# yoxu515/aot-benchmark

Hardware: NVIDIA H100
Metric: frames/sec (480p, 10 obj) (higher is better)
Workload: dtype f32

## Files before the change

aot_benchmark_b200/csrc/attn_tc.cuh:

```cuda
#pragma once
#include "common.cuh"
#include "tc_common.cuh"

namespace aotb {
namespace tc {

constexpr float AT_LOG2E = 1.4426950408889634f;

struct AttnTcArgs {
    int N, Tk;
    const int* Tk_dev;
    float* O;
    int ldo;
    float* Opart;
    float* Mpart;
    float* Lpart;
    int splits;
    int split_unit;
    int spin;
    float* dbg;
};

template <int QC, int VC, int STAGES, int BK, int NWG>
struct AttnSmem {
    static constexpr int BM = 64 * NWG;
    static constexpr int Q_BYTES = QC * BM * 128;
    static constexpr int K_BYTES = QC * BK * 128;
    static constexpr int V_BYTES = VC * BK * 128;
    static constexpr int STAGE_BYTES = K_BYTES + V_BYTES;
    static constexpr int TOTAL = Q_BYTES + STAGES * STAGE_BYTES + (1 + 2 * STAGES) * 8 + 1024;
};

template <int N>
__device__ __forceinline__ void wgmma_ss(float* d, uint64_t a, uint64_t b, uint32_t scale_d) {
    if (N == 128) wgmma_ss_n128(d, a, b, scale_d);
    else wgmma_ss_n64(d, a, b, scale_d);
}

template <int QC, int VC, int STAGES, bool EXACT, int BK, int NWG, bool AHEAD>
__global__ void __launch_bounds__(32 * (4 * NWG + 1), NWG == 1 ? 2 : 1)
attn_tc_kernel(const __grid_constant__ CUtensorMap tmQ, const __grid_constant__ CUtensorMap tmK,
               const __grid_constant__ CUtensorMap tmV, const AttnTcArgs a) {
    using SM = AttnSmem<QC, VC, STAGES, BK, NWG>;
    constexpr int BM = SM::BM, TMA_WARP = 4 * NWG, SR = BK / 2;
    extern __shared__ uint8_t smem_raw[];
    uint8_t* smem = reinterpret_cast<uint8_t*>((reinterpret_cast<uintptr_t>(smem_raw) + 1023) & ~(uintptr_t)1023);
    uint8_t* sQ = smem;
    uint8_t* sKV = smem + SM::Q_BYTES;
    uint64_t* q_full = reinterpret_cast<uint64_t*>(sKV + STAGES * SM::STAGE_BYTES);
    uint64_t* kv_full = q_full + 1;
    uint64_t* kv_free = kv_full + STAGES;

    const int tid = threadIdx.x, warp = tid >> 5, lane = tid & 31;
    const int qt = blockIdx.x, y = blockIdx.y, z = blockIdx.z;
    const int qc0 = QC == 1 ? y : 0, vc0 = y * VC;
    pdl_trigger();
    if (tid == 0) {
        mbar_init(q_full, 1);
        for (int s = 0; s < STAGES; ++s) { mbar_init(&kv_full[s], 1); mbar_init(&kv_free[s], 4 * NWG); }
        fence_mbar_init();
    }
    __syncthreads();
    pdl_wait();

    const int tk = a.Tk_dev ? *a.Tk_dev : a.Tk;
    const int units = (tk + a.split_unit - 1) / a.split_unit;
    const int per = (units + a.splits - 1) / a.splits;
    const int k0 = min(z * per * a.split_unit, tk), k1 = min((z + 1) * per * a.split_unit, tk);
    const int ntiles = (k1 - k0 + BK - 1) / BK;

    if (warp == TMA_WARP) {
        if (elect_one() && ntiles > 0) {
            tma_prefetch_desc(&tmQ); tma_prefetch_desc(&tmK); tma_prefetch_desc(&tmV);
            mbar_arrive_expect_tx(q_full, SM::Q_BYTES);
            for (int c = 0; c < QC; ++c) tma_load_3d(sQ + c * BM * 128, &tmQ, q_full, 0, qt * BM, qc0 + c);
            for (int n = 0; n < ntiles; ++n) {
                const int s = n % STAGES;
                if (n >= STAGES) mbar_wait(&kv_free[s], ((n / STAGES) - 1) & 1);
                uint8_t* st = sKV + s * SM::STAGE_BYTES;
                mbar_arrive_expect_tx(&kv_full[s], SM::STAGE_BYTES);
                const int key0 = k0 + n * BK;
                for (int c = 0; c < QC; ++c) tma_load_3d(st + c * BK * 128, &tmK, &kv_full[s], 0, key0, qc0 + c);
                for (int v = 0; v < VC; ++v)
                    tma_load_3d(st + SM::K_BYTES + v * BK * 128, &tmV, &kv_full[s], 0, key0, vc0 + v);
            }
        }
        return;
    }

    const int wg = warp >> 2, wq = warp & 3;
    const int row0 = wg * 64 + wq * 16 + (lane >> 2);
    const int cq = (lane & 3) * 2;
    float m[2] = {-INFINITY, -INFINITY}, l[2] = {0.f, 0.f};
    float o[VC][32];
#pragma unroll
    for (int v = 0; v < VC; ++v)
#pragma unroll
        for (int j = 0; j < 32; ++j) o[v][j] = 0.f;
    const bool dump = a.dbg && blockIdx.x == 0 && blockIdx.y == 0 && blockIdx.z == 0;
    const uint64_t dQ = smem_desc_sw128(smem_u32(sQ + wg * 64 * 128));
    const uint64_t dKV0 = smem_desc_sw128(smem_u32(sKV));
    if (ntiles > 0) mbar_wait_cp(q_full, 0, a.spin);

    auto issue_s = [&](int n, float* sc) {
        const uint64_t dK = dKV0 + (uint64_t)(((n % STAGES) * SM::STAGE_BYTES) >> 4);
        wgmma_fence();
#pragma unroll
        for (int c = 0; c < QC; ++c) {
            const uint64_t q = dQ + (uint64_t)((c * BM * 128) >> 4), k = dK + (uint64_t)((c * BK * 128) >> 4);
#pragma unroll
            for (int ks = 0; ks < 2; ++ks) {
                wgmma_ss<BK>(sc, q + 2 * ks, k + 2 * ks, (c | ks) ? 1u : 0u);
                if (EXACT) {
                    wgmma_ss<BK>(sc, q + 4 + 2 * ks, k + 2 * ks, 1u);
                    wgmma_ss<BK>(sc, q + 2 * ks, k + 4 + 2 * ks, 1u);
                }
            }
        }
        wgmma_commit();
    };
    float sbuf[AHEAD ? 2 : 1][SR];
    if (AHEAD && ntiles > 0) {
        mbar_wait_cp(&kv_full[0], 0, a.spin);
        issue_s(0, sbuf[0]);
    }

#pragma unroll 1
    for (int n = 0; n < ntiles; ++n) {
        const int s = n % STAGES;
        float* sc = sbuf[0];
        if (AHEAD) {
            if (n + 1 < ntiles) {
                mbar_wait_cp(&kv_full[(n + 1) % STAGES], ((n + 1) / STAGES) & 1, a.spin);
                issue_s(n + 1, sbuf[AHEAD ? 1 : 0]);
                wgmma_wait<1>();
            } else {
                wgmma_wait<0>();
            }
        } else {
            mbar_wait_cp(&kv_full[s], (n / STAGES) & 1, a.spin);
            issue_s(n, sc);
            wgmma_wait<0>();
        }
        reg_fence<SR>(sc);
        const uint64_t dV = dKV0 + (uint64_t)((s * SM::STAGE_BYTES + SM::K_BYTES) >> 4);
        const int key0 = k0 + n * BK;
        if (dump && key0 < 128) {
#pragma unroll
            for (int j = 0; j < SR; ++j) {
                const int key = key0 + 8 * (j >> 2) + cq + (j & 1);
                if (key < 128) a.dbg[(row0 + 8 * ((j >> 1) & 1)) * 128 + key] = sc[j];
            }
        }
        if (key0 + BK > k1) {
#pragma unroll
            for (int j = 0; j < SR; ++j)
                if (key0 + 8 * (j >> 2) + cq + (j & 1) >= k1) sc[j] = -INFINITY;
        }
        float mx[2] = {m[0], m[1]};
#pragma unroll
        for (int j = 0; j < SR; ++j) mx[(j >> 1) & 1] = fmaxf(mx[(j >> 1) & 1], sc[j]);
#pragma unroll
        for (int h = 0; h < 2; ++h) {
            mx[h] = fmaxf(mx[h], __shfl_xor_sync(0xffffffffu, mx[h], 1));
            mx[h] = fmaxf(mx[h], __shfl_xor_sync(0xffffffffu, mx[h], 2));
        }
        float f[2], neg[2];
#pragma unroll
        for (int h = 0; h < 2; ++h) {
            f[h] = mx[h] > m[h] ? ex2((m[h] - mx[h]) * AT_LOG2E) : 1.f;
            m[h] = mx[h];
            l[h] *= f[h];
            neg[h] = m[h] * AT_LOG2E;
        }
#pragma unroll
        for (int v = 0; v < VC; ++v)
#pragma unroll
            for (int j = 0; j < 32; ++j) o[v][j] *= f[(j >> 1) & 1];
        uint32_t ph[SR / 2], pl[SR / 2];
#pragma unroll
        for (int j = 0; j < SR; j += 2) {
            const int h = (j >> 1) & 1;
            const float p0 = ex2(fmaf(sc[j], AT_LOG2E, -neg[h])), p1 = ex2(fmaf(sc[j + 1], AT_LOG2E, -neg[h]));
            l[h] += p0 + p1;
            const __half2 hi = __floats2half2_rn(p0, p1);
            ph[j >> 1] = *reinterpret_cast<const uint32_t*>(&hi);
            if (EXACT) pl[j >> 1] = cvt_h2(p0 - __low2float(hi), p1 - __high2float(hi));
        }
        wgmma_fence();
#pragma unroll
        for (int v = 0; v < VC; ++v) {
            const uint64_t vd = dV + (uint64_t)((v * BK * 128) >> 4);
#pragma unroll
            for (int kk = 0; kk < BK / 16; ++kk) {
                wgmma_rs_n64_tb(o[v], ph + 4 * kk, vd + (uint64_t)(kk * 128));
                if (EXACT) wgmma_rs_n64_tb(o[v], pl + 4 * kk, vd + (uint64_t)(kk * 128));
            }
        }
        wgmma_commit();
        wgmma_wait<0>();
#pragma unroll
        for (int v = 0; v < VC; ++v) reg_fence<32>(o[v]);
        mbar_arrive_warp(&kv_free[s]);
        if (AHEAD) {
            reg_fence<SR>(sbuf[AHEAD ? 1 : 0]);
#pragma unroll
            for (int j = 0; j < SR; ++j) sbuf[0][j] = sbuf[AHEAD ? 1 : 0][j];
        }
    }

#pragma unroll
    for (int h = 0; h < 2; ++h) {
        l[h] += __shfl_xor_sync(0xffffffffu, l[h], 1);
        l[h] += __shfl_xor_sync(0xffffffffu, l[h], 2);
    }
    if (dump) {
#pragma unroll
        for (int j = 0; j < 32; ++j) a.dbg[128 * 128 + (row0 + 8 * ((j >> 1) & 1)) * 64 + 8 * (j >> 2) + cq + (j & 1)] = o[0][j];
    }
    const int cols = gridDim.y * VC * 32;
#pragma unroll
    for (int h = 0; h < 2; ++h) {
        const int q = qt * BM + row0 + 8 * h;
        if (q >= a.N) continue;
        const float inv = 1.f / l[h];
#pragma unroll
        for (int v = 0; v < VC; ++v) {
#pragma unroll
            for (int g = 0; g < 4; ++g) {
                const int j = 4 * g + 2 * h;
                float2 r = make_float2(o[v][j] + o[v][j + 16], o[v][j + 1] + o[v][j + 17]);
                const int col = (vc0 + v) * 32 + 8 * g + cq;
                if (a.splits == 1) {
                    r.x *= inv; r.y *= inv;
                    *reinterpret_cast<float2*>(a.O + (size_t)q * a.ldo + col) = r;
                } else {
                    *reinterpret_cast<float2*>(a.Opart + ((size_t)z * a.N + q) * cols + col) = r;
                }
            }
        }
        if (a.splits > 1 && (lane & 3) == 0 && (QC == 1 || y == 0)) {
            const size_t idx = ((size_t)z * (QC == 1 ? gridDim.y : 1) + (QC == 1 ? y : 0)) * a.N + q;
            a.Mpart[idx] = m[h];
            a.Lpart[idx] = l[h];
        }
    }
}

template <int QC, int VC, int STAGES, int BK, int NWG, bool AHEAD>
int launch_attn_tc(const CUtensorMap& tq, const CUtensorMap& tk, const CUtensorMap& tv, const AttnTcArgs& a, dim3 grid,
                   int exact, cudaStream_t st, const char* what) {
    constexpr int smem = AttnSmem<QC, VC, STAGES, BK, NWG>::TOTAL;
    auto kt = attn_tc_kernel<QC, VC, STAGES, true, BK, NWG, AHEAD>;
    auto kf = attn_tc_kernel<QC, VC, STAGES, false, BK, NWG, AHEAD>;
    static bool configured = false;
    if (!configured) {
        cudaError_t e = cudaFuncSetAttribute(kt, cudaFuncAttributeMaxDynamicSharedMemorySize, smem);
        if (e == cudaSuccess) e = cudaFuncSetAttribute(kf, cudaFuncAttributeMaxDynamicSharedMemorySize, smem);
        if (e != cudaSuccess) {
            set_error("%s: cudaFuncSetAttribute: %s", what, cudaGetErrorString(e));
            return AOTB_ERR_CUDA;
        }
        configured = true;
    }
    launch(exact ? kt : kf, grid, dim3(32 * (4 * NWG + 1)), smem, st, tq, tk, tv, a);
    return check_launch(what);
}

}
}
```

aot_benchmark_b200/csrc/tc_common.cuh:

```cuda
#pragma once
#include <cuda.h>
#include <cuda_fp16.h>
#include <cuda_runtime.h>
#include <cstdint>

namespace aotb {
namespace tc {

__device__ __forceinline__ uint32_t smem_u32(const void* p) { return (uint32_t)__cvta_generic_to_shared(p); }

__device__ __forceinline__ bool elect_one() {
    uint32_t pred;
    asm volatile(
        "{\n\t.reg .pred P;\n\telect.sync _|P, 0xffffffff;\n\tselp.b32 %0, 1, 0, P;\n\t}\n" : "=r"(pred));
    return pred != 0;
}

__device__ __forceinline__ void mbar_init(uint64_t* bar, uint32_t count) {
    asm volatile("mbarrier.init.shared::cta.b64 [%0], %1;" ::"r"(smem_u32(bar)), "r"(count) : "memory");
}
__device__ __forceinline__ void fence_mbar_init() { asm volatile("fence.mbarrier_init.release.cluster;" ::: "memory"); }
__device__ __forceinline__ void mbar_arrive_warp(uint64_t* bar) {
    __syncwarp();
    if ((threadIdx.x & 31) == 0) asm volatile("mbarrier.arrive.shared::cta.b64 _, [%0];" ::"r"(smem_u32(bar)) : "memory");
}
__device__ __forceinline__ void mbar_arrive(uint64_t* bar) {
    asm volatile("mbarrier.arrive.shared::cta.b64 _, [%0];" ::"r"(smem_u32(bar)) : "memory");
}
__device__ __forceinline__ void mbar_arrive_expect_tx(uint64_t* bar, uint32_t bytes) {
    asm volatile("mbarrier.arrive.expect_tx.shared::cta.b64 _, [%0], %1;" ::"r"(smem_u32(bar)), "r"(bytes) : "memory");
}
__device__ __forceinline__ void mbar_wait(uint64_t* bar, uint32_t parity) {
    const uint32_t addr = smem_u32(bar);
    uint32_t done = 0;
    uint32_t spins = 0;
    while (true) {
        asm volatile(
            "{\n\t.reg .pred P;\n\tmbarrier.try_wait.parity.shared::cta.b64 P, [%1], %2, %3;\n\tselp.b32 %0, 1, 0, P;\n\t}\n"
            : "=r"(done)
            : "r"(addr), "r"(parity), "r"(20000u)
            : "memory");
        if (done) break;
        if (++spins > (1u << 24)) __trap();
    }
}

__device__ __forceinline__ void mbar_wait_spin(uint64_t* bar, uint32_t parity) {
    const uint32_t addr = smem_u32(bar);
    uint32_t done = 0;
    uint32_t spins = 0;
    while (true) {
        asm volatile(
            "{\n\t.reg .pred P;\n\tmbarrier.try_wait.parity.shared::cta.b64 P, [%1], %2;\n\tselp.b32 %0, 1, 0, P;\n\t}\n"
            : "=r"(done)
            : "r"(addr), "r"(parity)
            : "memory");
        if (done) break;
        if (++spins > (1u << 28)) __trap();
    }
}

__device__ __forceinline__ void mbar_wait_cp(uint64_t* bar, uint32_t parity, int spin) {
    if (spin) mbar_wait_spin(bar, parity);
    else mbar_wait(bar, parity);
}

__device__ __forceinline__ void tma_prefetch_desc(const CUtensorMap* m) {
    asm volatile("prefetch.tensormap [%0];" ::"l"(reinterpret_cast<uint64_t>(m)) : "memory");
}
__device__ __forceinline__ void tma_load_2d(void* dst, const CUtensorMap* m, uint64_t* bar, int c0, int c1) {
    asm volatile(
        "cp.async.bulk.tensor.2d.shared::cluster.global.mbarrier::complete_tx::bytes [%0], [%1, {%3, %4}], [%2];"
        ::"r"(smem_u32(dst)), "l"(reinterpret_cast<uint64_t>(m)), "r"(smem_u32(bar)), "r"(c0), "r"(c1)
        : "memory");
}
__device__ __forceinline__ void tma_load_3d(void* dst, const CUtensorMap* m, uint64_t* bar, int c0, int c1, int c2) {
    asm volatile(
        "cp.async.bulk.tensor.3d.shared::cluster.global.mbarrier::complete_tx::bytes [%0], [%1, {%3, %4, %5}], [%2];"
        ::"r"(smem_u32(dst)), "l"(reinterpret_cast<uint64_t>(m)), "r"(smem_u32(bar)), "r"(c0), "r"(c1), "r"(c2)
        : "memory");
}
__device__ __forceinline__ void fence_proxy_async() { asm volatile("fence.proxy.async.shared::cta;" ::: "memory"); }

__device__ __forceinline__ uint64_t smem_desc_sw128(uint32_t saddr) {
    uint64_t d = 0;
    d |= (uint64_t)((saddr & 0x3FFFF) >> 4);
    d |= (uint64_t)1 << 16;
    d |= (uint64_t)(1024 >> 4) << 32;
    d |= (uint64_t)1 << 62;
    return d;
}
__device__ __forceinline__ void wgmma_fence() { asm volatile("wgmma.fence.sync.aligned;" ::: "memory"); }
__device__ __forceinline__ void wgmma_commit() { asm volatile("wgmma.commit_group.sync.aligned;" ::: "memory"); }
template <int N>
__device__ __forceinline__ void wgmma_wait() { asm volatile("wgmma.wait_group.sync.aligned %0;" ::"n"(N) : "memory"); }
template <int R>
__device__ __forceinline__ void reg_fence(float* d) {
#pragma unroll
    for (int i = 0; i < R; ++i) asm volatile("" : "+f"(d[i])::"memory");
}

__device__ __forceinline__ void wgmma_ss_n64(float* d, uint64_t a_desc, uint64_t b_desc, uint32_t scale_d) {
    asm volatile(
        "{\n\t.reg .pred p;\n\tsetp.ne.b32 p, %34, 0;\n\t"
        "wgmma.mma_async.sync.aligned.m64n64k16.f32.f16.f16 "
        "{%0, %1, %2, %3, %4, %5, %6, %7, %8, %9, %10, %11, %12, %13, %14, %15, "
        "%16, %17, %18, %19, %20, %21, %22, %23, %24, %25, %26, %27, %28, %29, %30, %31}, "
        "%32, %33, p, 1, 1, 0, 0;\n\t}\n"
        : "+f"(d[0]), "+f"(d[1]), "+f"(d[2]), "+f"(d[3]), "+f"(d[4]), "+f"(d[5]), "+f"(d[6]), "+f"(d[7]),
          "+f"(d[8]), "+f"(d[9]), "+f"(d[10]), "+f"(d[11]), "+f"(d[12]), "+f"(d[13]), "+f"(d[14]), "+f"(d[15]),
          "+f"(d[16]), "+f"(d[17]), "+f"(d[18]), "+f"(d[19]), "+f"(d[20]), "+f"(d[21]), "+f"(d[22]), "+f"(d[23]),
          "+f"(d[24]), "+f"(d[25]), "+f"(d[26]), "+f"(d[27]), "+f"(d[28]), "+f"(d[29]), "+f"(d[30]), "+f"(d[31])
        : "l"(a_desc), "l"(b_desc), "r"(scale_d));
}

__device__ __forceinline__ void wgmma_ss_n128(float* d, uint64_t a_desc, uint64_t b_desc, uint32_t scale_d) {
    asm volatile(
        "{\n\t.reg .pred p;\n\tsetp.ne.b32 p, %66, 0;\n\t"
        "wgmma.mma_async.sync.aligned.m64n128k16.f32.f16.f16 "
        "{%0, %1, %2, %3, %4, %5, %6, %7, %8, %9, %10, %11, %12, %13, %14, %15, "
        "%16, %17, %18, %19, %20, %21, %22, %23, %24, %25, %26, %27, %28, %29, %30, %31, "
        "%32, %33, %34, %35, %36, %37, %38, %39, %40, %41, %42, %43, %44, %45, %46, %47, "
        "%48, %49, %50, %51, %52, %53, %54, %55, %56, %57, %58, %59, %60, %61, %62, %63}, "
        "%64, %65, p, 1, 1, 0, 0;\n\t}\n"
        : "+f"(d[0]), "+f"(d[1]), "+f"(d[2]), "+f"(d[3]), "+f"(d[4]), "+f"(d[5]), "+f"(d[6]), "+f"(d[7]),
          "+f"(d[8]), "+f"(d[9]), "+f"(d[10]), "+f"(d[11]), "+f"(d[12]), "+f"(d[13]), "+f"(d[14]), "+f"(d[15]),
          "+f"(d[16]), "+f"(d[17]), "+f"(d[18]), "+f"(d[19]), "+f"(d[20]), "+f"(d[21]), "+f"(d[22]), "+f"(d[23]),
          "+f"(d[24]), "+f"(d[25]), "+f"(d[26]), "+f"(d[27]), "+f"(d[28]), "+f"(d[29]), "+f"(d[30]), "+f"(d[31]),
          "+f"(d[32]), "+f"(d[33]), "+f"(d[34]), "+f"(d[35]), "+f"(d[36]), "+f"(d[37]), "+f"(d[38]), "+f"(d[39]),
          "+f"(d[40]), "+f"(d[41]), "+f"(d[42]), "+f"(d[43]), "+f"(d[44]), "+f"(d[45]), "+f"(d[46]), "+f"(d[47]),
          "+f"(d[48]), "+f"(d[49]), "+f"(d[50]), "+f"(d[51]), "+f"(d[52]), "+f"(d[53]), "+f"(d[54]), "+f"(d[55]),
          "+f"(d[56]), "+f"(d[57]), "+f"(d[58]), "+f"(d[59]), "+f"(d[60]), "+f"(d[61]), "+f"(d[62]), "+f"(d[63])
        : "l"(a_desc), "l"(b_desc), "r"(scale_d));
}

__device__ __forceinline__ void wgmma_ss_n256(float* d, uint64_t a_desc, uint64_t b_desc, uint32_t scale_d) {
    asm volatile(
        "{\n\t.reg .pred p;\n\tsetp.ne.b32 p, %130, 0;\n\t"
        "wgmma.mma_async.sync.aligned.m64n256k16.f32.f16.f16 "
        "{%0, %1, %2, %3, %4, %5, %6, %7, %8, %9, %10, %11, %12, %13, %14, %15, "
        "%16, %17, %18, %19, %20, %21, %22, %23, %24, %25, %26, %27, %28, %29, %30, %31, "
        "%32, %33, %34, %35, %36, %37, %38, %39, %40, %41, %42, %43, %44, %45, %46, %47, "
        "%48, %49, %50, %51, %52, %53, %54, %55, %56, %57, %58, %59, %60, %61, %62, %63, "
        "%64, %65, %66, %67, %68, %69, %70, %71, %72, %73, %74, %75, %76, %77, %78, %79, "
        "%80, %81, %82, %83, %84, %85, %86, %87, %88, %89, %90, %91, %92, %93, %94, %95, "
        "%96, %97, %98, %99, %100, %101, %102, %103, %104, %105, %106, %107, %108, %109, %110, %111, "
        "%112, %113, %114, %115, %116, %117, %118, %119, %120, %121, %122, %123, %124, %125, %126, %127}, "
        "%128, %129, p, 1, 1, 0, 0;\n\t}\n"
        : "+f"(d[0]), "+f"(d[1]), "+f"(d[2]), "+f"(d[3]), "+f"(d[4]), "+f"(d[5]), "+f"(d[6]), "+f"(d[7]),
          "+f"(d[8]), "+f"(d[9]), "+f"(d[10]), "+f"(d[11]), "+f"(d[12]), "+f"(d[13]), "+f"(d[14]), "+f"(d[15]),
          "+f"(d[16]), "+f"(d[17]), "+f"(d[18]), "+f"(d[19]), "+f"(d[20]), "+f"(d[21]), "+f"(d[22]), "+f"(d[23]),
          "+f"(d[24]), "+f"(d[25]), "+f"(d[26]), "+f"(d[27]), "+f"(d[28]), "+f"(d[29]), "+f"(d[30]), "+f"(d[31]),
          "+f"(d[32]), "+f"(d[33]), "+f"(d[34]), "+f"(d[35]), "+f"(d[36]), "+f"(d[37]), "+f"(d[38]), "+f"(d[39]),
          "+f"(d[40]), "+f"(d[41]), "+f"(d[42]), "+f"(d[43]), "+f"(d[44]), "+f"(d[45]), "+f"(d[46]), "+f"(d[47]),
          "+f"(d[48]), "+f"(d[49]), "+f"(d[50]), "+f"(d[51]), "+f"(d[52]), "+f"(d[53]), "+f"(d[54]), "+f"(d[55]),
          "+f"(d[56]), "+f"(d[57]), "+f"(d[58]), "+f"(d[59]), "+f"(d[60]), "+f"(d[61]), "+f"(d[62]), "+f"(d[63]),
          "+f"(d[64]), "+f"(d[65]), "+f"(d[66]), "+f"(d[67]), "+f"(d[68]), "+f"(d[69]), "+f"(d[70]), "+f"(d[71]),
          "+f"(d[72]), "+f"(d[73]), "+f"(d[74]), "+f"(d[75]), "+f"(d[76]), "+f"(d[77]), "+f"(d[78]), "+f"(d[79]),
          "+f"(d[80]), "+f"(d[81]), "+f"(d[82]), "+f"(d[83]), "+f"(d[84]), "+f"(d[85]), "+f"(d[86]), "+f"(d[87]),
          "+f"(d[88]), "+f"(d[89]), "+f"(d[90]), "+f"(d[91]), "+f"(d[92]), "+f"(d[93]), "+f"(d[94]), "+f"(d[95]),
          "+f"(d[96]), "+f"(d[97]), "+f"(d[98]), "+f"(d[99]), "+f"(d[100]), "+f"(d[101]), "+f"(d[102]), "+f"(d[103]),
          "+f"(d[104]), "+f"(d[105]), "+f"(d[106]), "+f"(d[107]), "+f"(d[108]), "+f"(d[109]), "+f"(d[110]), "+f"(d[111]),
          "+f"(d[112]), "+f"(d[113]), "+f"(d[114]), "+f"(d[115]), "+f"(d[116]), "+f"(d[117]), "+f"(d[118]), "+f"(d[119]),
          "+f"(d[120]), "+f"(d[121]), "+f"(d[122]), "+f"(d[123]), "+f"(d[124]), "+f"(d[125]), "+f"(d[126]), "+f"(d[127])
        : "l"(a_desc), "l"(b_desc), "r"(scale_d));
}

__device__ __forceinline__ void wgmma_rs_n64_tb(float* d, const uint32_t* a, uint64_t b_desc) {
    asm volatile(
        "{\n\t.reg .pred p;\n\tsetp.ne.b32 p, 1, 0;\n\t"
        "wgmma.mma_async.sync.aligned.m64n64k16.f32.f16.f16 "
        "{%0, %1, %2, %3, %4, %5, %6, %7, %8, %9, %10, %11, %12, %13, %14, %15, "
        "%16, %17, %18, %19, %20, %21, %22, %23, %24, %25, %26, %27, %28, %29, %30, %31}, "
        "{%32, %33, %34, %35}, %36, p, 1, 1, 1;\n\t}\n"
        : "+f"(d[0]), "+f"(d[1]), "+f"(d[2]), "+f"(d[3]), "+f"(d[4]), "+f"(d[5]), "+f"(d[6]), "+f"(d[7]),
          "+f"(d[8]), "+f"(d[9]), "+f"(d[10]), "+f"(d[11]), "+f"(d[12]), "+f"(d[13]), "+f"(d[14]), "+f"(d[15]),
          "+f"(d[16]), "+f"(d[17]), "+f"(d[18]), "+f"(d[19]), "+f"(d[20]), "+f"(d[21]), "+f"(d[22]), "+f"(d[23]),
          "+f"(d[24]), "+f"(d[25]), "+f"(d[26]), "+f"(d[27]), "+f"(d[28]), "+f"(d[29]), "+f"(d[30]), "+f"(d[31])
        : "r"(a[0]), "r"(a[1]), "r"(a[2]), "r"(a[3]), "l"(b_desc));
}


__device__ __forceinline__ float ex2(float x) {
    float y;
    asm("ex2.approx.ftz.f32 %0, %1;" : "=f"(y) : "f"(x));
    return y;
}
__device__ __forceinline__ uint32_t cvt_h2(float lo, float hi) {
    uint32_t r;
    asm("cvt.rn.f16x2.f32 %0, %1, %2;" : "=r"(r) : "f"(hi), "f"(lo));
    return r;
}

__device__ __forceinline__ void cluster_sync_all() {
    asm volatile("barrier.cluster.arrive.release.aligned;\n\tbarrier.cluster.wait.acquire.aligned;" ::: "memory");
}
__device__ __forceinline__ uint32_t dsmem_addr(uint32_t local_saddr, uint32_t cta_rank) {
    uint32_t r;
    asm volatile("mapa.shared::cluster.u32 %0, %1, %2;" : "=r"(r) : "r"(local_saddr), "r"(cta_rank));
    return r;
}
__device__ __forceinline__ float4 dsmem_ld_f4(uint32_t cluster_saddr) {
    float4 v;
    asm volatile("ld.shared::cluster.v4.f32 {%0, %1, %2, %3}, [%4];"
                 : "=f"(v.x), "=f"(v.y), "=f"(v.z), "=f"(v.w)
                 : "r"(cluster_saddr));
    return v;
}

typedef CUresult (*PFN_encodeTiled)(CUtensorMap*, CUtensorMapDataType, cuuint32_t, void*, const cuuint64_t*,
                                    const cuuint64_t*, const cuuint32_t*, const cuuint32_t*, CUtensorMapInterleave,
                                    CUtensorMapSwizzle, CUtensorMapL2promotion, CUtensorMapFloatOOBfill);
PFN_encodeTiled tensor_map_encoder();

int make_tmap_rows64(CUtensorMap* out, const void* base, int rows, int heads, int box_rows);

}
}
```

Before: 362.3.

## Add FA3-style intra-warpgroup softmax/GEMM pipelining with ping-pong warpgroup scheduling

For the QC=1, VC=1, BK=64, NWG=2 non-AHEAD configuration, the attention loop is restructured so each step issues the next tile's QK^T GEMM and the current tile's PV GEMM together. The softmax and exp/pack for the next tile then runs while the PV GEMM is in flight, with P fragments double-buffered in registers. Named barriers make the two warpgroups take turns issuing tensor-core work, so one warpgroup's softmax overlaps the other's GEMMs. The intent is to hide softmax latency behind tensor-core work, at the cost of more register pressure and extra barrier synchronisation. The row-sum rescale is folded into the exp accumulation.

Result: faster. 367.9, median of 6 (+1.5%).

```diff
diff --git a/aot_benchmark_b200/csrc/attn_tc.cuh b/aot_benchmark_b200/csrc/attn_tc.cuh
--- a/aot_benchmark_b200/csrc/attn_tc.cuh
+++ b/aot_benchmark_b200/csrc/attn_tc.cuh
@@ -43,6 +43,7 @@
                const __grid_constant__ CUtensorMap tmV, const AttnTcArgs a) {
     using SM = AttnSmem<QC, VC, STAGES, BK, NWG>;
     constexpr int BM = SM::BM, TMA_WARP = 4 * NWG, SR = BK / 2;
+    constexpr bool PIPE = QC == 1 && VC == 1 && BK == 64 && NWG == 2 && !AHEAD;
     extern __shared__ uint8_t smem_raw[];
     uint8_t* smem = reinterpret_cast<uint8_t*>((reinterpret_cast<uintptr_t>(smem_raw) + 1023) & ~(uintptr_t)1023);
     uint8_t* sQ = smem;
@@ -119,93 +120,211 @@
         }
         wgmma_commit();
     };
-    float sbuf[AHEAD ? 2 : 1][SR];
-    if (AHEAD && ntiles > 0) {
-        mbar_wait_cp(&kv_full[0], 0, a.spin);
-        issue_s(0, sbuf[0]);
-    }
-
+    if constexpr (PIPE) {
+        auto row_max = [&](int n, float* sc, float* f, float* neg) {
+            const int key0 = k0 + n * BK;
+            if (dump && key0 < 128) {
+#pragma unroll
+                for (int j = 0; j < SR; ++j) {
+                    const int key = key0 + 8 * (j >> 2) + cq + (j & 1);
+                    if (key < 128) a.dbg[(row0 + 8 * ((j >> 1) & 1)) * 128 + key] = sc[j];
+                }
+            }
+            if (key0 + BK > k1) {
+#pragma unroll
+                for (int j = 0; j < SR; ++j)
+                    if (key0 + 8 * (j >> 2) + cq + (j & 1) >= k1) sc[j] = -INFINITY;
+            }
+            float mx[2] = {m[0], m[1]};
+#pragma unroll
+            for (int j = 0; j < SR; ++j) mx[(j >> 1) & 1] = fmaxf(mx[(j >> 1) & 1], sc[j]);
+#pragma unroll
+            for (int h = 0; h < 2; ++h) {
+                mx[h] = fmaxf(mx[h], __shfl_xor_sync(0xffffffffu, mx[h], 1));
+                mx[h] = fmaxf(mx[h], __shfl_xor_sync(0xffffffffu, mx[h], 2));
+            }
+#pragma unroll
+            for (int h = 0; h < 2; ++h) {
+                f[h] = mx[h] > m[h] ? ex2((m[h] - mx[h]) * AT_LOG2E) : 1.f;
+                m[h] = mx[h];
+                neg[h] = m[h] * AT_LOG2E;
+            }
+        };
+        auto rescale_o = [&](const float* f) {
+#pragma unroll
+            for (int v = 0; v < VC; ++v)
+#pragma unroll
+                for (int j = 0; j < 32; ++j) o[v][j] *= f[(j >> 1) & 1];
+        };
+        auto exp_pack = [&](const float* sc, const float* f, const float* neg, uint32_t* ph, uint32_t* pl) {
+#pragma unroll
+            for (int j = 0; j < SR; j += 2) {
+                const int h = (j >> 1) & 1;
+                const float p0 = ex2(fmaf(sc[j], AT_LOG2E, -neg[h])), p1 = ex2(fmaf(sc[j + 1], AT_LOG2E, -neg[h]));
+                l[h] = j < 4 ? __fmaf_rn(l[h], f[h], __fadd_rn(p0, p1)) : __fadd_rn(l[h], __fadd_rn(p0, p1));
+                const __half2 hi = __floats2half2_rn(p0, p1);
+                ph[j >> 1] = *reinterpret_cast<const uint32_t*>(&hi);
+                if (EXACT) pl[j >> 1] = cvt_h2(p0 - __low2float(hi), p1 - __high2float(hi));
+            }
+        };
+        auto v_desc = [&](int s) { return dKV0 + (uint64_t)((s * SM::STAGE_BYTES + SM::K_BYTES) >> 4); };
+        auto issue_pv = [&](uint64_t dV, const uint32_t* ph, const uint32_t* pl) {
+            wgmma_fence();
+#pragma unroll
+            for (int v = 0; v < VC; ++v) {
+                const uint64_t vd = dV + (uint64_t)((v * BK * 128) >> 4);
+#pragma unroll
+                for (int kk = 0; kk < BK / 16; ++kk) {
+                    wgmma_rs_n64_tb(o[v], ph + 4 * kk, vd + (uint64_t)(kk * 128));
+                    if (EXACT) wgmma_rs_n64_tb(o[v], pl + 4 * kk, vd + (uint64_t)(kk * 128));
+                }
+            }
+            wgmma_commit();
+        };
+
+        auto turn_begin = [&]() { named_bar_sync(1 + wg, 256); };
+        auto turn_end = [&]() { named_bar_arrive(2 - wg, 256); };
+        float sc[SR], f[2], neg[2];
+        uint32_t ph0[SR / 2], pl0[SR / 2], ph1[SR / 2], pl1[SR / 2];
+        auto step = [&](int n, uint32_t* ph, uint32_t* pl, uint32_t* phn, uint32_t* pln) {
+            mbar_wait_cp(&kv_full[(n + 1) % STAGES], ((n + 1) / STAGES) & 1, a.spin);
+            turn_begin();
+            issue_s(n + 1, sc);
+            issue_pv(v_desc(n % STAGES), ph, pl);
+            turn_end();
+            wgmma_wait<1>();
+            reg_fence<SR>(sc);
+            row_max(n + 1, sc, f, neg);
+            exp_pack(sc, f, neg, phn, pln);
+            wgmma_wait<0>();
+            reg_fence<32>(o[0]);
+            reg_fence<SR / 2>(ph);
+            if (EXACT) reg_fence<SR / 2>(pl);
+            mbar_arrive_warp(&kv_free[n % STAGES]);
+            rescale_o(f);
+        };
+        auto last = [&](int n, const uint32_t* ph, const uint32_t* pl) {
+            turn_begin();
+            issue_pv(v_desc(n % STAGES), ph, pl);
+            turn_end();
+            wgmma_wait<0>();
+            reg_fence<32>(o[0]);
+            mbar_arrive_warp(&kv_free[n % STAGES]);
+        };
+        if (ntiles > 0) {
+            if (wg == 1) turn_end();
+            mbar_wait_cp(&kv_full[0], 0, a.spin);
+            turn_begin();
+            issue_s(0, sc);
+            turn_end();
+            wgmma_wait<0>();
+            reg_fence<SR>(sc);
+            row_max(0, sc, f, neg);
+            rescale_o(f);
+            exp_pack(sc, f, neg, ph0, pl0);
+            int n = 0;
 #pragma unroll 1
-    for (int n = 0; n < ntiles; ++n) {
-        const int s = n % STAGES;
-        float* sc = sbuf[0];
-        if (AHEAD) {
+            for (; n + 2 < ntiles; n += 2) {
+                step(n, ph0, pl0, ph1, pl1);
+                step(n + 1, ph1, pl1, ph0, pl0);
+            }
             if (n + 1 < ntiles) {
-                mbar_wait_cp(&kv_full[(n + 1) % STAGES], ((n + 1) / STAGES) & 1, a.spin);
-                issue_s(n + 1, sbuf[AHEAD ? 1 : 0]);
-                wgmma_wait<1>();
+                step(n, ph0, pl0, ph1, pl1);
+                last(n + 1, ph1, pl1);
             } else {
+                last(n, ph0, pl0);
+            }
+            if (wg == 0) turn_begin();
+        }
+    } else {
+        float sbuf[AHEAD ? 2 : 1][SR];
+        if (AHEAD && ntiles > 0) {
+            mbar_wait_cp(&kv_full[0], 0, a.spin);
+            issue_s(0, sbuf[0]);
+        }
+
+#pragma unroll 1
+        for (int n = 0; n < ntiles; ++n) {
+            const int s = n % STAGES;
+            float* sc = sbuf[0];
+            if (AHEAD) {
+                if (n + 1 < ntiles) {
+                    mbar_wait_cp(&kv_full[(n + 1) % STAGES], ((n + 1) / STAGES) & 1, a.spin);
+                    issue_s(n + 1, sbuf[AHEAD ? 1 : 0]);
+                    wgmma_wait<1>();
+                } else {
+                    wgmma_wait<0>();
+                }
+            } else {
+                mbar_wait_cp(&kv_full[s], (n / STAGES) & 1, a.spin);
+                issue_s(n, sc);
                 wgmma_wait<0>();
             }
-        } else {
-            mbar_wait_cp(&kv_full[s], (n / STAGES) & 1, a.spin);
-            issue_s(n, sc);
+            reg_fence<SR>(sc);
+            const uint64_t dV = dKV0 + (uint64_t)((s * SM::STAGE_BYTES + SM::K_BYTES) >> 4);
+            const int key0 = k0 + n * BK;
+            if (dump && key0 < 128) {
+#pragma unroll
+                for (int j = 0; j < SR; ++j) {
+                    const int key = key0 + 8 * (j >> 2) + cq + (j & 1);
+                    if (key < 128) a.dbg[(row0 + 8 * ((j >> 1) & 1)) * 128 + key] = sc[j];
+                }
+            }
+            if (key0 + BK > k1) {
+#pragma unroll
+                for (int j = 0; j < SR; ++j)
+                    if (key0 + 8 * (j >> 2) + cq + (j & 1) >= k1) sc[j] = -INFINITY;
+            }
+            float mx[2] = {m[0], m[1]};
+#pragma unroll
+            for (int j = 0; j < SR; ++j) mx[(j >> 1) & 1] = fmaxf(mx[(j >> 1) & 1], sc[j]);
+#pragma unroll
+            for (int h = 0; h < 2; ++h) {
+                mx[h] = fmaxf(mx[h], __shfl_xor_sync(0xffffffffu, mx[h], 1));
+                mx[h] = fmaxf(mx[h], __shfl_xor_sync(0xffffffffu, mx[h], 2));
+            }
+            float f[2], neg[2];
+#pragma unroll
+            for (int h = 0; h < 2; ++h) {
+                f[h] = mx[h] > m[h] ? ex2((m[h] - mx[h]) * AT_LOG2E) : 1.f;
+                m[h] = mx[h];
+                l[h] *= f[h];
+                neg[h] = m[h] * AT_LOG2E;
+            }
+#pragma unroll
+            for (int v = 0; v < VC; ++v)
+#pragma unroll
+                for (int j = 0; j < 32; ++j) o[v][j] *= f[(j >> 1) & 1];
+            uint32_t ph[SR / 2], pl[SR / 2];
+#pragma unroll
+            for (int j = 0; j < SR; j += 2) {
+                const int h = (j >> 1) & 1;
+                const float p0 = ex2(fmaf(sc[j], AT_LOG2E, -neg[h])), p1 = ex2(fmaf(sc[j + 1], AT_LOG2E, -neg[h]));
+                l[h] += p0 + p1;
+                const __half2 hi = __floats2half2_rn(p0, p1);
+                ph[j >> 1] = *reinterpret_cast<const uint32_t*>(&hi);
+                if (EXACT) pl[j >> 1] = cvt_h2(p0 - __low2float(hi), p1 - __high2float(hi));
+            }
+            wgmma_fence();
+#pragma unroll
+            for (int v = 0; v < VC; ++v) {
+                const uint64_t vd = dV + (uint64_t)((v * BK * 128) >> 4);
+#pragma unroll
+                for (int kk = 0; kk < BK / 16; ++kk) {
+                    wgmma_rs_n64_tb(o[v], ph + 4 * kk, vd + (uint64_t)(kk * 128));
+                    if (EXACT) wgmma_rs_n64_tb(o[v], pl + 4 * kk, vd + (uint64_t)(kk * 128));
+                }
+            }
+            wgmma_commit();
             wgmma_wait<0>();
-        }
-        reg_fence<SR>(sc);
-        const uint64_t dV = dKV0 + (uint64_t)((s * SM::STAGE_BYTES + SM::K_BYTES) >> 4);
-        const int key0 = k0 + n * BK;
-        if (dump && key0 < 128) {
-#pragma unroll
-            for (int j = 0; j < SR; ++j) {
-                const int key = key0 + 8 * (j >> 2) + cq + (j & 1);
-                if (key < 128) a.dbg[(row0 + 8 * ((j >> 1) & 1)) * 128 + key] = sc[j];
-            }
-        }
-        if (key0 + BK > k1) {
-#pragma unroll
-            for (int j = 0; j < SR; ++j)
-                if (key0 + 8 * (j >> 2) + cq + (j & 1) >= k1) sc[j] = -INFINITY;
-        }
-        float mx[2] = {m[0], m[1]};
-#pragma unroll
-        for (int j = 0; j < SR; ++j) mx[(j >> 1) & 1] = fmaxf(mx[(j >> 1) & 1], sc[j]);
-#pragma unroll
-        for (int h = 0; h < 2; ++h) {
-            mx[h] = fmaxf(mx[h], __shfl_xor_sync(0xffffffffu, mx[h], 1));
-            mx[h] = fmaxf(mx[h], __shfl_xor_sync(0xffffffffu, mx[h], 2));
-        }
-        float f[2], neg[2];
-#pragma unroll
-        for (int h = 0; h < 2; ++h) {
-            f[h] = mx[h] > m[h] ? ex2((m[h] - mx[h]) * AT_LOG2E) : 1.f;
-            m[h] = mx[h];
-            l[h] *= f[h];
-            neg[h] = m[h] * AT_LOG2E;
-        }
-#pragma unroll
-        for (int v = 0; v < VC; ++v)
-#pragma unroll
-            for (int j = 0; j < 32; ++j) o[v][j] *= f[(j >> 1) & 1];
-        uint32_t ph[SR / 2], pl[SR / 2];
-#pragma unroll
-        for (int j = 0; j < SR; j += 2) {
-            const int h = (j >> 1) & 1;
-            const float p0 = ex2(fmaf(sc[j], AT_LOG2E, -neg[h])), p1 = ex2(fmaf(sc[j + 1], AT_LOG2E, -neg[h]));
-            l[h] += p0 + p1;
-            const __half2 hi = __floats2half2_rn(p0, p1);
-            ph[j >> 1] = *reinterpret_cast<const uint32_t*>(&hi);
-            if (EXACT) pl[j >> 1] = cvt_h2(p0 - __low2float(hi), p1 - __high2float(hi));
-        }
-        wgmma_fence();
-#pragma unroll
-        for (int v = 0; v < VC; ++v) {
-            const uint64_t vd = dV + (uint64_t)((v * BK * 128) >> 4);
-#pragma unroll
-            for (int kk = 0; kk < BK / 16; ++kk) {
-                wgmma_rs_n64_tb(o[v], ph + 4 * kk, vd + (uint64_t)(kk * 128));
-                if (EXACT) wgmma_rs_n64_tb(o[v], pl + 4 * kk, vd + (uint64_t)(kk * 128));
-            }
-        }
-        wgmma_commit();
-        wgmma_wait<0>();
-#pragma unroll
-        for (int v = 0; v < VC; ++v) reg_fence<32>(o[v]);
-        mbar_arrive_warp(&kv_free[s]);
-        if (AHEAD) {
-            reg_fence<SR>(sbuf[AHEAD ? 1 : 0]);
-#pragma unroll
-            for (int j = 0; j < SR; ++j) sbuf[0][j] = sbuf[AHEAD ? 1 : 0][j];
+#pragma unroll
+            for (int v = 0; v < VC; ++v) reg_fence<32>(o[v]);
+            mbar_arrive_warp(&kv_free[s]);
+            if (AHEAD) {
+                reg_fence<SR>(sbuf[AHEAD ? 1 : 0]);
+#pragma unroll
+                for (int j = 0; j < SR; ++j) sbuf[0][j] = sbuf[AHEAD ? 1 : 0][j];
+            }
         }
     }
 
diff --git a/aot_benchmark_b200/csrc/tc_common.cuh b/aot_benchmark_b200/csrc/tc_common.cuh
--- a/aot_benchmark_b200/csrc/tc_common.cuh
+++ b/aot_benchmark_b200/csrc/tc_common.cuh
@@ -65,6 +65,13 @@
     else mbar_wait(bar, parity);
 }
 
+__device__ __forceinline__ void named_bar_sync(uint32_t id, uint32_t threads) {
+    asm volatile("bar.sync %0, %1;" ::"r"(id), "r"(threads) : "memory");
+}
+__device__ __forceinline__ void named_bar_arrive(uint32_t id, uint32_t threads) {
+    asm volatile("bar.arrive %0, %1;" ::"r"(id), "r"(threads) : "memory");
+}
+
 __device__ __forceinline__ void tma_prefetch_desc(const CUtensorMap* m) {
     asm volatile("prefetch.tensormap [%0];" ::"l"(reinterpret_cast<uint64_t>(m)) : "memory");
 }
@@ -98,6 +105,11 @@
 __device__ __forceinline__ void reg_fence(float* d) {
 #pragma unroll
     for (int i = 0; i < R; ++i) asm volatile("" : "+f"(d[i])::"memory");
+}
+template <int R>
+__device__ __forceinline__ void reg_fence(uint32_t* a) {
+#pragma unroll
+    for (int i = 0; i < R; ++i) asm volatile("" : "+r"(a[i])::"memory");
 }
 
 __device__ __forceinline__ void wgmma_ss_n64(float* d, uint64_t a_desc, uint64_t b_desc, uint32_t scale_d) {
```
